# mitiko/weath3rb0i

Hardware: AMD Instinct MI355X
Metric: encode MiB/s, 64 KiB blocks, bit-exact vs CPU ref (higher is better)
Workload: dtype u32

## Files before the change

### weath3rb0i_amd/csrc/w3_predict.h

```cpp
#pragma once
#include "w3_device.h"
#include "../../include/w3hip.h"

namespace w3 {

#define W3_PF 8

#define W3_HALF_CU_LDS 81920u
template <int NW, size_t USED> struct HalfCuPad { static constexpr size_t words = (NW > 1 && USED < W3_HALF_CU_LDS) ? (W3_HALF_CU_LDS - USED + 3u) / 4u : (NW > 1 ? 0u : 1u); };
template <size_t WORDS> struct HalfCuPadDecl {
    static __device__ __forceinline__ void keep(uint64_t n) {
        __shared__ uint32_t pad_[WORDS];
        if (n == ~0ull) pad_[threadIdx.x % WORDS] = 1u;
    }
};
template <> struct HalfCuPadDecl<0> { static __device__ __forceinline__ void keep(uint64_t) {} };
#define W3_HALF_CU_PAD(NW, USED) HalfCuPadDecl<((NW) > 1 ? HalfCuPad<NW, (USED)>::words : 0u)>::keep(a.n);

struct PredictArgs {
    const uint8_t *in;
    uint64_t n;
    uint32_t block_size, nblocks;
    uint4 *P;
    const uint2 *keys;
// ... 29 lines not shown
}

template <int H>
__device__ __forceinline__ void match_windows(uint32_t w16, uint64_t M[8]) {
    uint64_t X[16];
#pragma unroll
    for (int b = 1; b < 16; b++) {
        if (b >= 1 && b <= 7 + H) {
            const bool mybit = (w16 >> b) & 1u;
            const uint64_t B = __ballot(mybit);
            X[b] = mybit ? B : ~B;
        }
    }
    if constexpr (H == 8) {
        uint64_t A2[15], A4[13];
#pragma unroll
        for (int b = 1; b <= 14; b++) A2[b] = X[b] & X[b + 1];
#pragma unroll
        for (int b = 1; b <= 12; b++) A4[b] = A2[b] & A2[b + 2];
#pragma unroll
        for (int j = 0; j < 8; j++) M[j] = A4[8 - j] & A4[12 - j];
    } else {
#pragma unroll
        for (int j = 0; j < 8; j++) {
            uint64_t m = ~0ull;
#pragma unroll
            for (int k = 0; k < H; k++) m &= X[8 - j + k];
            M[j] = m;
        }
    }
}

template <int H>
__device__ __forceinline__ void match_keys(uint2 k8, uint64_t M[8]) {
#pragma unroll
    for (int j = 0; j < 8; j++) {
        const uint32_t key = ((j < 4 ? k8.x : k8.y) >> (8 * (j & 3))) & 0xFFu;
        uint32_t mlo = 0xFFFFFFFFu, mhi = 0xFFFFFFFFu;
#pragma unroll
        for (int k = 0; k < H; k++) {
            const uint32_t sm = (uint32_t)__builtin_amdgcn_sbfe((int)key, k, 1);
            const uint64_t B = __ballot(sm != 0u);
            mlo &= ~((uint32_t)B ^ sm);
            mhi &= ~((uint32_t)(B >> 32) ^ sm);
        }
        M[j] = ((uint64_t)mhi << 32) | mlo;
    }
}

__device__ __forceinline__ uint32_t mbcnt64(uint64_t m) {
    return __builtin_amdgcn_mbcnt_hi((uint32_t)(m >> 32), __builtin_amdgcn_mbcnt_lo((uint32_t)m, 0u));
}

template <bool GROUPED>
__device__ __forceinline__ void rank_round(uint32_t c0, const uint32_t key[8], const uint64_t M[8], uint64_t seg, bool valid, bool rd,
                                           uint32_t *tbl, uint32_t p[8], uint32_t fin[8], uint32_t &wmask) {
    __asm__ volatile("" ::: "memory");
    const uint64_t gt = lane_gt_mask();
    const int lane = threadIdx.x & 63;
    wmask = 0u;
    uint32_t basev[8];
#pragma unroll
    for (int j = 0; j < 8; j++) basev[j] = tbl[j * 256 + key[j]];
#pragma unroll
    for (int j = 0; j < 8; j++) {
        const uint64_t Mj = M[j] & seg;
        const uint32_t bit = (c0 >> (7 - j)) & 1u;
        const uint64_t ones = __ballot(bit) & Mj;
        uint32_t base = basev[j];
        if constexpr (GROUPED) base = rd ? base : 0u;
        const uint32_t b0 = base & 0xFFFFu, b1 = base >> 16;
        const uint32_t n1l = mbcnt64(ones), n0l = mbcnt64(Mj) - n1l;
        uint32_t s0 = b0 + n0l, s1 = b1 + n1l;
        const bool last = valid && (Mj & gt) == 0ull;
        uint32_t f0 = s0 + (bit ^ 1u), f1 = s1 + bit;
        uint64_t satm = __ballot(last && (f0 >= 65535u || f1 >= 65535u));
        uint32_t f = f0 | (f1 << 16);
        while (satm) {
            const int k = __ffsll((long long)satm) - 1;
            const uint64_t Mc = readlane_u64(Mj, k);
            const uint64_t Oc = readlane_u64(ones, k);
            uint32_t st = readlane_u32(base, k);
            uint64_t it = Mc;
            while (it) {
                const int m = __ffsll((long long)it) - 1;
                it &= it - 1;
                if (lane == m) { s0 = st & 0xFFFFu; s1 = st >> 16; }
                st = counter_update_packed(st, (uint32_t)(Oc >> m) & 1u);
            }
            if (lane == k) f = st;
            satm &= satm - 1;
        }
        p[j] = counter_p(s0, s1);
        fin[j] = f;
        wmask |= last ? (1u << j) : 0u;
    }
    if constexpr (!GROUPED) {
#pragma unroll
        for (int j = 0; j < 8; j++)
            if ((wmask >> j) & 1u) tbl[j * 256 + key[j]] = fin[j];
        __asm__ volatile("" ::: "memory");
    }
}

#define W3_ATOMIC_LIM 65400u
#ifndef W3_ATOMIC_MAXSEG
#define W3_ATOMIC_MAXSEG 4u
#endif
typedef uint16_t w3_u16x2 __attribute__((ext_vector_type(2)));

__device__ __forceinline__ void atomic_round(uint32_t *tbl, uint32_t c0, const uint32_t key[8], bool on, uint32_t v[8]) {
#pragma unroll
    for (int j = 0; j < 8; j++) {
        const uint32_t inc = on ? (((c0 >> (7 - j)) & 1u) ? 0x10000u : 1u) : 0u;
        v[j] = __hip_atomic_fetch_add(&tbl[j * 256 + key[j]], inc, __ATOMIC_RELAXED, __HIP_MEMORY_SCOPE_WORKGROUP);
    }
}
__device__ __forceinline__ bool atomic_round_hot(const uint32_t v[8]) {
    w3_u16x2 m = __builtin_bit_cast(w3_u16x2, v[0]);
#pragma unroll
    for (int j = 1; j < 8; j++) m = __builtin_elementwise_max(m, __builtin_bit_cast(w3_u16x2, v[j]));
    return __ballot(max((uint32_t)m.x, (uint32_t)m.y) >= W3_ATOMIC_LIM) != 0ull;
}

__host__ __device__ __forceinline__ uint32_t lds_order_hash(uint32_t wave, uint32_t round, uint32_t lane) {
    uint32_t x = (wave * 64u + round) * 64u + lane + 0x9E3779B9u;
    x ^= x >> 16; x *= 0x7FEB352Du; x ^= x >> 15; x *= 0x846CA68Bu; x ^= x >> 16;
    return x;
}
__host__ __device__ __forceinline__ uint32_t lds_order_key(uint32_t wave, uint32_t h) {
    const uint32_t kind = wave & 3u;
    return kind == 0 ? 77u : kind == 1 ? (h & 7u) * 32u + 1u : kind == 2 ? (h & 255u) : (h & 2047u);
}
__global__ void __launch_bounds__(64) k_lds_order_selftest(uint32_t *old) {
    __shared__ uint32_t tbl[2048];
    const uint32_t lane = threadIdx.x;
    for (uint32_t i = lane; i < 2048u; i += 64u) tbl[i] = 0u;
    __builtin_amdgcn_wave_barrier();
    for (uint32_t r = 0; r < 32u; r++) {
        const uint32_t h = lds_order_hash(blockIdx.x, r, lane);
        old[(blockIdx.x * 32u + r) * 64u + lane] =
            __hip_atomic_fetch_add(&tbl[lds_order_key(blockIdx.x, h)], (h >> 20) & 1u ? 0x10000u : 1u, __ATOMIC_RELAXED, __HIP_MEMORY_SCOPE_WORKGROUP);
    }
}

__device__ __forceinline__ uint4 pack_p(const uint32_t p[8]) {
    return make_uint4(p[0] | (p[1] << 16), p[2] | (p[3] << 16), p[4] | (p[5] << 16), p[6] | (p[7] << 16));
}

__device__ __forceinline__ uint32_t mix_pair(uint32_t cur, uint32_t nw) {
    const uint32_t c_lo = cur & 0xFFFFu, c_hi = cur >> 16, n_lo = nw & 0xFFFFu, n_hi = nw >> 16;
    const uint32_t lo = opinion_dist(n_lo) > opinion_dist(c_lo) ? n_lo : c_lo;
    const uint32_t hi = opinion_dist(n_hi) > opinion_dist(c_hi) ? n_hi : c_hi;
    return lo | (hi << 16);
// ... 56 lines not shown
            uint2 k8 = make_uint2(0, 0);
            if constexpr (KEYS) k8 = st_k[rr * 64u + lane];
            uint32_t c0 = 0, key[8], p[8];
            if constexpr (KEYS) {
                c0 = valid ? w : 0u;
#pragma unroll
                for (int j = 0; j < 8; j++) key[j] = ((j < 4 ? k8.x : k8.y) >> (8 * (j & 3))) & KM;
            } else {
                const uint32_t wv = valid ? w : 0u;
                c0 = wv & 0xFFu;
#pragma unroll
                for (int j = 0; j < 8; j++) key[j] = ((wv & 0xFFFFu) >> (8 - j)) & KM;
            }
            if (!exact) {
                uint32_t v[8];
                __asm__ volatile("" ::: "memory");
                atomic_round(tbl, c0, key, valid, v);
                __asm__ volatile("" ::: "memory");
                if ((a.dbg_flags & 8u) && base == 64u && (a.fault_block == 0xFFFFFFFFu || a.fault_block == b)) v[0] = (uint32_t)__shfl_xor((int)v[0], 1, 64);
#pragma unroll
                for (int j = 0; j < 8; j++) p[j] = counter_p_packed(v[j]);
                exact = atomic_round_hot(v);
            } else {
                uint64_t M[8];
                if constexpr (KEYS) match_keys<H>(valid ? k8 : make_uint2(0, 0), M);
                else match_windows<H>((valid ? w : 0u) & 0xFFFFu, M);
                const uint64_t seg = __ballot(valid);
                uint32_t fin[8], wm;
                rank_round<false>(c0, key, M, seg, valid, true, tbl, p, fin, wm);
            }
            {
                uint4 *dst = valid ? a.P + (off + i) : a.sink + lane;
                *dst = pack_p(p);
            }
          }
        }
    }
}

__device__ __forceinline__ uint32_t wave_excl_scan_u32(uint32_t v, uint32_t *total) {
    const int lane = threadIdx.x & 63;
    uint32_t inc = v;
#pragma unroll
    for (int d = 1; d < 64; d <<= 1) {
        uint32_t o = __shfl_up(inc, d, 64);
        if (lane >= d) inc += o;
    }
    *total = __shfl(inc, 63, 64);
    return inc - v;
}


template <int NPASS, bool C2ONLY = false>
__device__ __forceinline__ void partition_hist(const uint8_t *blk, uint32_t len, uint32_t first, uint32_t *hist) {
    const int lane = threadIdx.x & 63;
    const uint64_t gt = lane_gt_mask();
    if (lane < 16 * NPASS) hist[lane] = 0u;
    __builtin_amdgcn_wave_barrier();
    uint32_t wn[W3_PF];
    const uint32_t last = len - 1u;
#pragma unroll
    for (int r = 0; r < W3_PF; r++) wn[r] = load_window(blk, min(r * 64u + lane, last), first);
    for (uint32_t base = 0; base < len; base += 64u * W3_PF) {
        uint32_t wc[W3_PF];
#pragma unroll
        for (int r = 0; r < W3_PF; r++) wc[r] = wn[r];
// ... 724 lines not shown
```

### weath3rb0i_amd/csrc/w3_twophase.h

```cpp
#pragma once
#include <hip/hip_runtime.h>

#include <algorithm>
#include <cstdlib>
#include <string>
#include <type_traits>
#include <vector>

#include "w3_apm.h"
#include "w3_coder.h"
#include "w3_coder4.h"
#include "w3_coder5.h"
#include "w3_predict.h"
#include "w3_predict_wave.h"
#include "w3_slot.h"
#include "w3_slot2.h"
#include "w3_spec.h"
#include "w3_tables_plan.h"

static inline const char *w3_tune_env(const char *name) {
#ifdef W3_TUNING
    return getenv(name);
#else
    (void)name;
    return nullptr;
#endif
}

enum { W3_VAR_NO_LDS_ATOMICS = 1, W3_VAR_PARTITION4 = 2, W3_VAR_NO_CHAINED_PARTITION = 4, W3_VAR_CM_UNSTAGED = 8, W3_VAR_NO_SIDE_STREAM = 16,
       W3_VAR_INJECT_LDS_FAULT = 32 ,
       W3_VAR_HALF_CU = 64    ,
       W3_VAR_FULL_CU = 128   ,
       W3_VAR_SLOT_TABLE = 256  ,
       W3_VAR_SLOT_SORTED = 512 ,
       W3_VAR_DECODE_LANE = 1024 ,
       W3_VAR_AOH_DECODE_SPEC = 2048  };

#define W3_SLOT_SORTED_MAX_BLOCKS 7000u

enum { W3_EV_PREDICT = 0, W3_EV_CODER = 1, W3_EV_PACK = 2, W3_EV_TOTAL = 3, W3_EV_APM = 4, W3_EV_SLOT = 5, W3_EV_ACHASH = 6,
       W3_EV_PART0 = 7 , W3_EV_RANK0 = 11 , W3_EV_SMALL = 15,
       W3_EV_SLOTS = 16 };
#define W3_NEV (2 * W3_EV_SLOTS)

struct TwoPhaseOptions {
    int coder_mode = 0;
    uint32_t acc_limit = 46;
    uint32_t variant = 0;
    uint32_t slot_budget_mb = 0;
    int verify = 1;
    uint32_t tune = 0;
    uint32_t fault_block = 0xFFFFFFFFu;
    uint32_t fault_kernels = 1u;
    int debug_stamps = 0;
};

struct TwoPhaseWs {
    void *P = nullptr, *keys = nullptr, *perm = nullptr, *redo = nullptr, *streams = nullptr, *rec = nullptr, *splits = nullptr;
    size_t P_cap = 0, keys_cap = 0, perm_cap = 0, redo_cap = 0, streams_cap = 0, rec_cap = 0, splits_cap = 0;
    w3::MixArgs mix{};
    bool P_valid = false;
    void *dbg = nullptr;
    bool achash_timed = false;
    hipEvent_t ev_pred_done = nullptr;
    int lds_order = -1;
    const int16_t *stretch = nullptr;
    const uint16_t *squash = nullptr;
    const uint2 *st = nullptr;
    const w3_huff_table *huff = nullptr;
    uint32_t *out_bits = nullptr;
    void *rec_w[4] = {nullptr, nullptr, nullptr, nullptr}, *perm_w[4] = {nullptr, nullptr, nullptr, nullptr}, *splits_w[4] = {nullptr, nullptr, nullptr, nullptr};
    size_t rec_w_cap[4] = {0, 0, 0, 0}, perm_w_cap[4] = {0, 0, 0, 0}, splits_w_cap[4] = {0, 0, 0, 0};
    int wide1_slot = -1;
    hipStream_t side = nullptr;
    struct PredictState {
        bool forked = false, lds_atomics = false;
        int n_def = 0, n_small_def = 0, n_live = 0;
        struct Deferred { w3::PredictArgs pa; int cls; uint32_t grid_rank; } deferred[4];
        uint64_t bytes = 0, slot_stride = 0;
        w3::SlotArgs sa;
    } pst;
    uint32_t *order_fault = nullptr;
    uint32_t *apm_oob = nullptr;
    bool half_cu = false;
    int n_wide = 0; bool small_timed = false;
    hipEvent_t ev_fork = nullptr, ev_join[4] = {nullptr, nullptr, nullptr, nullptr}, ev_small = nullptr;
    void *achash_lut = nullptr;
    size_t achash_lut_cap = 0;
    void *dummy = nullptr;
    size_t dummy_cap = 0;
    void *slot_tables = nullptr;
    size_t slot_tables_cap = 0;
    void *keys32 = nullptr; size_t keys32_cap = 0;
    void *slot_keys = nullptr; size_t slot_keys_cap = 0;
    bool slot_sorted = false;
    void *wave_tables = nullptr; size_t wave_tables_cap = 0;
    void *huff_redo = nullptr;
    size_t huff_redo_cap = 0;
    TwoPhaseOptions opt;
    uint64_t verify_calls = 0;
    TwoPhaseWs *vws = nullptr;
    void *vin = nullptr; size_t vin_cap = 0;
    bool used_lds_atomics = false;
    hipStream_t vstream = nullptr; hipEvent_t ev_v0 = nullptr, ev_v1 = nullptr;
    bool ext_streams = false;
    void release() {
        if (vws) { vws->release(); delete vws; vws = nullptr; }
        if (vin) (void)hipFree(vin);
        vin = nullptr; vin_cap = 0;
        if (vstream && !ext_streams) (void)hipStreamDestroy(vstream);
        if (ev_v0) (void)hipEventDestroy(ev_v0);
        if (ev_v1) (void)hipEventDestroy(ev_v1);
        vstream = nullptr; ev_v0 = ev_v1 = nullptr;
        if (P) (void)hipFree(P);
        if (keys) (void)hipFree(keys);
        if (perm) (void)hipFree(perm);
        if (redo) (void)hipFree(redo);
        for (int w = 0; w < 4; w++) {
            if (rec_w[w]) (void)hipFree(rec_w[w]);
            if (perm_w[w]) (void)hipFree(perm_w[w]);
            if (splits_w[w]) (void)hipFree(splits_w[w]);
            rec_w[w] = perm_w[w] = splits_w[w] = nullptr; rec_w_cap[w] = perm_w_cap[w] = splits_w_cap[w] = 0;
        }
        if (side && !ext_streams) (void)hipStreamDestroy(side);
        if (ev_fork) (void)hipEventDestroy(ev_fork);
        for (int w = 0; w < 4; w++) { if (ev_join[w]) (void)hipEventDestroy(ev_join[w]); ev_join[w] = nullptr; }
        if (ev_small) (void)hipEventDestroy(ev_small);
        ev_small = nullptr;
        side = nullptr; ev_fork = nullptr;
        if (ev_pred_done) (void)hipEventDestroy(ev_pred_done);
        ev_pred_done = nullptr;
        if (achash_lut) (void)hipFree(achash_lut);
// ... 47 lines not shown
}

static inline bool twophase_supported(const ParsedSpec &ps, size_t block_size, size_t n) {
    if (block_size > (1u << 24) || n < 8) return false;
    int n_slot = 0;
    for (int l = 0; l < ps.n_leaves; l++) n_slot += ps.leaf[l].kind == W3_NODE_SLOT_STATE;
    if (n_slot > W3_MAX_SLOT_LEAVES) return false;
    for (int l = 0; l < ps.n_leaves; l++)
        if (leaf_class(ps.leaf[l]) == LEAF_NONE) return false;
    return true;
}

#define W3_NW_SMALL 8
#define W3_NW_PART 4
#define W3_NW_RANK 6
#define W3_NW_RANK8 8
#define W3_HALF_CU_GRID 256u

template <bool KEYS, int NW = 1>
static inline void launch_small(int H, dim3 grid, hipStream_t s, const w3::PredictArgs &pa) {
    const dim3 blk(64 * NW);
    switch (H) {
    case 0: hipLaunchKernelGGL((w3::k_predict_small<0, KEYS, NW>), grid, blk, 0, s, pa); break;
    case 1: hipLaunchKernelGGL((w3::k_predict_small<1, KEYS, NW>), grid, blk, 0, s, pa); break;
    case 2: hipLaunchKernelGGL((w3::k_predict_small<2, KEYS, NW>), grid, blk, 0, s, pa); break;
    case 3: hipLaunchKernelGGL((w3::k_predict_small<3, KEYS, NW>), grid, blk, 0, s, pa); break;
    case 4: hipLaunchKernelGGL((w3::k_predict_small<4, KEYS, NW>), grid, blk, 0, s, pa); break;
    case 5: hipLaunchKernelGGL((w3::k_predict_small<5, KEYS, NW>), grid, blk, 0, s, pa); break;
    case 6: hipLaunchKernelGGL((w3::k_predict_small<6, KEYS, NW>), grid, blk, 0, s, pa); break;
    case 7: hipLaunchKernelGGL((w3::k_predict_small<7, KEYS, NW>), grid, blk, 0, s, pa); break;
    default: hipLaunchKernelGGL((w3::k_predict_small<8, KEYS, NW>), grid, blk, 0, s, pa); break;
    }
}
static inline void launch_small_shaped(const TwoPhaseWs &ws, int H, uint32_t nb, hipStream_t s, const w3::PredictArgs &pa) {
    if (ws.half_cu && (ws.opt.tune & 32u)) launch_small<false, W3_NW_SMALL>(H, dim3(std::min<uint32_t>((nb + W3_NW_SMALL - 1) / W3_NW_SMALL, 2 * W3_HALF_CU_GRID)), s, pa);
    else launch_small<false>(H, dim3(std::min<uint32_t>(nb, 256 * 20)), s, pa);
}

static inline int twophase_mix(TwoPhaseWs &ws, hipStream_t s, size_t n, std::string &err) {
    if (ws.P_valid) return W3_OK;
    int rc = tp_ensure(ws.P, ws.P_cap, n * 16, err);
    if (rc) return rc;
    ws.mix.P = (uint4 *)ws.P; ws.mix.n = n;
    hipLaunchKernelGGL(w3::k_mix, dim3(256 * 8), dim3(256), 0, s, ws.mix);
    hipError_t e = hipGetLastError();
    if (e != hipSuccess) { err = std::string("mix launch: ") + hipGetErrorString(e); return W3_E_HIP; }
    ws.P_valid = true;
    return W3_OK;
}

static inline bool twophase_lds_order_ok(TwoPhaseWs &ws, hipStream_t s) {
    if (ws.lds_order >= 0) return ws.lds_order == 1;
    ws.lds_order = 0;
    if (ws.opt.variant & W3_VAR_NO_LDS_ATOMICS) return false;
    const uint32_t waves = 64, rounds = 32, n = waves * rounds * 64;
    uint32_t *d_old = nullptr;
    if (hipMalloc(&d_old, (size_t)n * 4) != hipSuccess) { (void)hipGetLastError(); return false; }
    std::vector<uint32_t> old(n), t(2048);
    hipLaunchKernelGGL(w3::k_lds_order_selftest, dim3(waves), dim3(64), 0, s, d_old);
    bool ok = hipGetLastError() == hipSuccess && hipMemcpyAsync(old.data(), d_old, (size_t)n * 4, hipMemcpyDeviceToHost, s) == hipSuccess &&
              hipStreamSynchronize(s) == hipSuccess;
    (void)hipFree(d_old);
    if (!ok) { (void)hipGetLastError(); return false; }
    for (uint32_t w = 0; w < waves && ok; w++) {
        std::fill(t.begin(), t.end(), 0u);
        for (uint32_t r = 0; r < rounds && ok; r++)
            for (uint32_t l = 0; l < 64; l++) {
                const uint32_t h = w3::lds_order_hash(w, r, l), k = w3::lds_order_key(w, h);
                if (old[(w * rounds + r) * 64 + l] != t[k]) { ok = false; break; }
                t[k] += (h >> 20) & 1u ? 0x10000u : 1u;
            }
    }
    ws.lds_order = ok ? 1 : 0;
    return ok;
}

template <int MODE, int NW>
static inline void launch_partition8(bool fault, dim3 grid, hipStream_t s, const w3::PredictArgs &pa) {
    if (fault) hipLaunchKernelGGL((w3::k_partition8<MODE, NW, true>), grid, dim3(64 * NW), 0, s, pa);
    else hipLaunchKernelGGL((w3::k_partition8<MODE, NW>), grid, dim3(64 * NW), 0, s, pa);
}
template <int NBYTES, int NW, int PF>
static inline void launch_rank(bool fault, dim3 grid, hipStream_t s, const w3::PredictArgs &pa) {
    if (fault) hipLaunchKernelGGL((w3::k_rank_sorted<NBYTES, NW, PF, true>), grid, dim3(64 * NW), 0, s, pa);
    else hipLaunchKernelGGL((w3::k_rank_sorted<NBYTES, NW, PF>), grid, dim3(64 * NW), 0, s, pa);
}

static inline int twophase_predict_a(TwoPhaseWs &ws, hipStream_t s, const ParsedSpec &ps, const uint8_t *d_in, size_t n, size_t block_size,
                                     uint32_t nb, hipEvent_t *ev, std::string &err, bool join_all = false) {
    int rc = W3_OK;
    ws.P_valid = false;
    ws.achash_timed = false;
    const bool lds_atomics = twophase_lds_order_ok(ws, s);
    ws.used_lds_atomics = false;
    const uint32_t grid_small = std::min<uint32_t>(nb, 256 * 20);
    const uint32_t grid_wide = std::min<uint32_t>(nb, 256 * 16);
    ws.n_wide = 0; ws.small_timed = false;
    bool need_keys = false, need_perm = false;
    for (int l = 0; l < ps.n_leaves; l++) {
        int c = leaf_class(ps.leaf[l]);
        need_keys |= c == LEAF_SMALL_AC || c == LEAF_SMALL_HUFF;
        need_perm |= c == LEAF_WIDE1 || c == LEAF_WIDE2;
    }
    if (need_keys && (rc = tp_ensure(ws.keys, ws.keys_cap, n * 8, err))) return rc;
    if (need_perm) {
        int nw = 0;
        for (int l = 0; l < ps.n_leaves; l++) { const int c = leaf_class(ps.leaf[l]); nw += c == LEAF_WIDE1 || c == LEAF_WIDE2; }
        if (nw > 4) { err = "more than 4 wide Counter leaves"; return W3_E_UNSUPPORTED; }
        for (int w = 0; w < nw; w++) {
            if ((rc = tp_ensure(ws.perm_w[w], ws.perm_w_cap[w], (size_t)grid_wide * 2 * block_size * 8, err))) return rc;
            if ((rc = tp_ensure(ws.rec_w[w], ws.rec_w_cap[w], n * 8, err))) return rc;
            if ((rc = tp_ensure(ws.splits_w[w], ws.splits_w_cap[w], (size_t)nb * (W3_SLICES + 1) * 4 + 64, err))) return rc;
        }
        if (!ws.side || !ws.ev_fork) {
            bool ok = (ws.side || hipStreamCreateWithFlags(&ws.side, hipStreamNonBlocking) == hipSuccess) && hipEventCreateWithFlags(&ws.ev_fork, hipEventDisableTiming) == hipSuccess;
            for (int w = 0; w < 4 && ok; w++) ok = hipEventCreateWithFlags(&ws.ev_join[w], hipEventDisableTiming) == hipSuccess;
            ok = ok && hipEventCreateWithFlags(&ws.ev_small, hipEventDisableTiming) == hipSuccess;
            if (!ok) { (void)hipGetLastError(); err = "side stream creation failed"; return W3_E_HIP; }
        }
    }

    int live[W3_MAX_LEAVES], n_live = 0;
    for (int l = 0; l < ps.n_leaves; l++)
        if (leaf_class(ps.leaf[l]) != LEAF_FROZEN) live[n_live++] = l;
    if (n_live > 1 && (rc = tp_ensure(ws.streams, ws.streams_cap, (size_t)n_live * n * 16, err))) return rc;
    if (n_live <= 1 && (rc = tp_ensure(ws.P, ws.P_cap, n * 16, err))) return rc;

    if ((rc = tp_ensure(ws.dummy, ws.dummy_cap, 2048, err))) return rc;
// ... 85 lines not shown
                }
                hipLaunchKernelGGL(w3::k_predict_wave<true>, dim3((unsigned)waves), dim3(64), 0, s, wa);
                bytes += n * (1 + 32 + 32);
            } else {
                hipLaunchKernelGGL(w3::k_predict_wave<false>, dim3((unsigned)waves), dim3(64), 0, s, wa);
            }
            bytes += n * (8 + 16 + 8 * 16);
            hipError_t e = hipGetLastError();
            if (e != hipSuccess) { err = std::string("wave predict launch: ") + hipGetErrorString(e); return W3_E_HIP; }
            continue;
        }
        pa.hbits = nd.bits - 3;
        pa.sink = (uint4 *)ws.dummy;
        pa.maxseg = W3_ATOMIC_MAXSEG;
        if (const char *ev_ = w3_tune_env("W3_ATOMIC_MAXSEG")) pa.maxseg = (uint32_t)std::max(0, atoi(ev_));
        if (!lds_atomics) pa.dbg_flags |= 2u;
        if (ws.opt.variant & W3_VAR_INJECT_LDS_FAULT) pa.dbg_flags |= (ws.opt.fault_kernels & 7u) << 3;
        pa.fault_block = ws.opt.fault_block;
        bytes += n * 17;
        if (c == LEAF_SMALL_AC) {
            w3::HashArgs ha;
            memset(&ha, 0, sizeof ha);
            ha.in = d_in; ha.n = n; ha.block_size = (uint32_t)block_size; ha.max_bits = nd.max_bits;
            ha.hmask = (1u << (nd.bits - 3)) - 1u; ha.keys = (uint2 *)ws.keys;
            memcpy(ha.table, nd.table, sizeof ha.table);
            if ((rc = tp_ensure(ws.achash_lut, ws.achash_lut_cap, (size_t)(8u << W3_ACHASH_LUT_BITS) * 18, err))) return rc;
            ha.lut = (uint4 *)ws.achash_lut;
            ha.lut_key = (uint16_t *)((uint8_t *)ws.achash_lut + (size_t)(8u << W3_ACHASH_LUT_BITS) * 16);
            if (ev && !achash_timed) (void)hipEventRecord(ev[2 * W3_EV_ACHASH], s);
            hipLaunchKernelGGL(w3::k_achash_lut, dim3((8u << W3_ACHASH_LUT_BITS) / 256), dim3(256), 0, s, ha);
            hipLaunchKernelGGL(w3::k_achash, dim3((unsigned)((n + 255) / 256)), dim3(256), 0, s, ha);
            if (ev && !achash_timed) { (void)hipEventRecord(ev[2 * W3_EV_ACHASH + 1], s); achash_timed = true; ws.achash_timed = true; }
            pa.keys = (const uint2 *)ws.keys;
            launch_small<true>(nd.bits - 3, dim3(grid_small), s, pa);
            bytes += n * 17;
        } else if (c == LEAF_SMALL_HUFF) {
            if (!ws.huff) { err = "HuffHistory tables not staged"; return W3_E_HIP; }
            w3::HuffKeyArgs hk;
            memset(&hk, 0, sizeof hk);
            hk.in = d_in; hk.n = n; hk.block_size = (uint32_t)block_size; hk.hmask = (1u << (nd.bits - 3)) - 1u;
            hk.tb = ws.huff + nd.reserved; hk.keys = (uint2 *)ws.keys;
            if ((rc = tp_ensure(ws.huff_redo, ws.huff_redo_cap, (size_t)nb * 4, err))) return rc;
            hk.redo = (uint32_t *)ws.huff_redo; hk.nblocks = nb;
            (void)hipMemsetAsync(ws.huff_redo, 0, (size_t)nb * 4, s);
            hipLaunchKernelGGL(w3::k_huffkeys<false>, dim3((unsigned)((n + 255) / 256)), dim3(256), 0, s, hk);
            hipLaunchKernelGGL(w3::k_huffkeys_fix<false>, dim3((nb + 63u) / 64u), dim3(64), 0, s, hk);
            pa.keys = (const uint2 *)ws.keys;
            launch_small<true>(nd.bits - 3, dim3(grid_small), s, pa);
            bytes += n * 17;
        } else if (c == LEAF_SMALL) {
            if (n_small_def < 8 && (!join_all || (ws.opt.tune & 2048u))) small_def[n_small_def++] = pa;
            else {
                const bool timed = ev && !ws.small_timed;
                if (timed) { (void)hipEventRecord(ev[2 * W3_EV_SMALL], s); ws.small_timed = true; }
                launch_small_shaped(ws, nd.bits - 3, nb, s, pa);
                if (timed) (void)hipEventRecord(ev[2 * W3_EV_SMALL + 1], s);
            }
        } else {
            const int w = n_def;
            pa.perm = (uint32_t *)ws.perm_w[w];
            if (ws.opt.debug_stamps) {
                if (!ws.dbg && hipMalloc(&ws.dbg, 64) != hipSuccess) ws.dbg = nullptr;
                if (ws.dbg) { (void)hipMemsetAsync(ws.dbg, 0, 64, s); pa.dbg = (unsigned long long *)ws.dbg; }
            }
            pa.rec = (uint2 *)ws.rec_w[w]; pa.splits = (uint32_t *)ws.splits_w[w];
            pa.job_counter = (uint32_t *)ws.splits_w[w] + (size_t)nb * (W3_SLICES + 1);
            (void)hipMemsetAsync(pa.job_counter, 0, 4, sp);
            if (const char *ev_ = w3_tune_env("W3_DEBUG_NOSTORE")) pa.dbg_flags = (uint32_t)atoi(ev_) & 5u;
            if (!lds_atomics) pa.dbg_flags |= 2u;
            uint32_t rank_waves = 2048u;
            if (const char *ev_ = w3_tune_env("W3_RANK_GRID")) rank_waves = (uint32_t)std::max(64, atoi(ev_));
            const uint32_t nw_rank = (ws.opt.tune & 32768u) ? W3_NW_RANK8 : W3_NW_RANK;
            const uint32_t grid_rank = (ws.half_cu && (w == 0 || (ws.opt.tune & (32u | 64u))) && !(ws.opt.tune & 8u)) ? std::min<uint32_t>((nb * W3_SLICES + nw_rank - 1) / nw_rank, W3_HALF_CU_GRID)
                                                              : std::min<uint32_t>(nb * W3_SLICES, rank_waves);
            const bool chained = c == LEAF_WIDE2 && ws.wide1_slot >= 0 && !(ws.opt.variant & W3_VAR_NO_CHAINED_PARTITION);
            if (chained) pa.rec_src = (const uint2 *)ws.rec_w[ws.wide1_slot];
            const bool p8 = lds_atomics && !(ws.opt.variant & W3_VAR_PARTITION4);
            const uint32_t grid_p8h = std::min<uint32_t>((nb + W3_NW_PART - 1) / W3_NW_PART, 2 * W3_HALF_CU_GRID);
            const bool p8h = p8 && ws.half_cu && (ws.opt.tune & 32u);
            if (ev && w < 4) (void)hipEventRecord(ev[2 * (W3_EV_PART0 + w)], sp);
            const bool f8 = (pa.dbg_flags & 32u) != 0u;
// ... 165 lines not shown
    if (tm) tm->predict_bytes = bytes;
    if (d_P) *d_P = (const uint16_t *)ws.P;
    return W3_OK;
}

static inline int twophase_predict(TwoPhaseWs &ws, hipStream_t s, const ParsedSpec &ps, const uint8_t *d_in, size_t n, size_t block_size,
                                   uint32_t nb, bool need_P, const uint16_t **d_P, hipEvent_t *ev, w3_timing *tm, std::string &err) {
    int rc = twophase_predict_a(ws, s, ps, d_in, n, block_size, nb, ev, err, false);
    if (rc) return rc;
    return twophase_predict_b(ws, s, ps, d_in, n, block_size, nb, need_P, d_P, ev, tm, err);
}

static inline int twophase_verify(TwoPhaseWs &ws, hipStream_t s, const ParsedSpec &ps, const uint8_t *d_in, size_t n, size_t block_size,
                                  uint32_t nb, uint32_t *d_mismatch, std::string &err) {
    if (!ws.opt.verify || !ws.used_lds_atomics || nb == 0) return W3_OK;
    const uint32_t S = w3::verify_sample_size(nb, block_size, (uint32_t)std::max(1, ws.opt.verify));
    const uint32_t rot = w3::verify_rotation(ws.verify_calls, nb, S);
    const uint64_t last_off = (uint64_t)w3::verify_block(rot, S - 1u, nb, S) * block_size;
    const size_t vn = (size_t)(S - 1u) * block_size + (size_t)std::min<uint64_t>(block_size, n - last_off);
    const uint8_t *vsrc = nullptr;
    int rc;
    if (nb == 1) vsrc = d_in;
    else {
        if ((rc = tp_ensure(ws.vin, ws.vin_cap, vn, err))) return rc;
        hipLaunchKernelGGL(w3::k_gather_blocks, dim3(std::min<uint32_t>((uint32_t)((block_size + 255) / 256), 64u), S), dim3(256), 0, s,
                           d_in, (uint64_t)n, (uint32_t)block_size, nb, S, rot, (uint8_t *)ws.vin);
        vsrc = (const uint8_t *)ws.vin;
    }
    if (!ws.vws) ws.vws = new TwoPhaseWs();
    TwoPhaseWs &v = *ws.vws;
    v.opt = TwoPhaseOptions();
    v.opt.variant = (ws.opt.variant | W3_VAR_NO_LDS_ATOMICS | W3_VAR_PARTITION4 | W3_VAR_NO_SIDE_STREAM) & ~(uint32_t)W3_VAR_INJECT_LDS_FAULT;
    v.opt.verify = 0; v.opt.slot_budget_mb = ws.opt.slot_budget_mb;
    v.lds_order = 0;
    v.stretch = ws.stretch; v.squash = ws.squash; v.st = ws.st; v.huff = ws.huff;
    ParsedSpec vps;
    int map[W3_MAX_LEAVES], nmap = 0;
    int live_idx = 0;
    for (int l = 0; l < ps.n_leaves; l++) {
        const int c = leaf_class(ps.leaf[l]);
        if (c == LEAF_FROZEN) continue;
        if (c != LEAF_SLOT && c != LEAF_WAVE) { vps.leaf[vps.n_leaves++] = ps.leaf[l]; map[nmap++] = live_idx; }
        live_idx++;
    }
    vps.n_huff = ps.n_huff; vps.huff = ps.huff;
    if (vps.n_leaves == 0) return W3_OK;
    if ((rc = twophase_predict(v, s, vps, vsrc, vn, block_size, (uint32_t)((vn + block_size - 1) / block_size), false, nullptr, nullptr, nullptr, err))) return rc;
    for (int k = 0; k < nmap; k++)
        hipLaunchKernelGGL(w3::k_compare_blocks, dim3(std::min<uint32_t>((uint32_t)((block_size + 255) / 256), 64u), S), dim3(256), 0, s,
                           ws.mix.src[map[k]], v.mix.src[k], (uint64_t)n, (uint32_t)block_size, nb, S, rot, d_mismatch);
    hipError_t e = hipGetLastError();
    if (e != hipSuccess) { err = std::string("verify launch: ") + hipGetErrorString(e); return W3_E_HIP; }
    return W3_OK;
}

static inline int twophase_apm(TwoPhaseWs &ws, hipStream_t s, const ParsedSpec &ps, const uint8_t *d_in, size_t n, size_t block_size,
                               uint32_t nb, hipEvent_t *ev, w3_timing *tm, std::string &err) {
    if (ps.n_apm == 0) return W3_OK;
    if (!ws.stretch || !ws.squash) { err = "APM LUTs not staged"; return W3_E_HIP; }
    int rc = tp_ensure(ws.P, ws.P_cap, n * 16, err);
    if (rc) return rc;
    if ((rc = tp_ensure(ws.dummy, ws.dummy_cap, 2048, err))) return rc;
    if (ev) (void)hipEventRecord(ev[2 * W3_EV_APM], s);
    uint64_t bytes = 0;
    bool partitioned = false;
    for (int k = 0; k < ps.n_apm; k++) {
        w3::ApmArgs aa;
// ... 198 lines not shown
```

### weath3rb0i_amd/csrc/w3hip.hip

```cpp
#include "../../include/w3hip.h"

#include <hip/hip_runtime.h>

#include <algorithm>
#include <cstddef>
#include <cstdio>
#include <cstring>
#include <mutex>
#include <string>
#include <thread>
#include <vector>

#include "w3_spec.h"
#include "w3_huff.h"
#include "w3_generic.h"
#include "w3_cm.h"
#include "w3_decode_spec.h"
#include "w3_pack.h"
#include "w3_tables_plan.h"
#include "w3_jobs.h"
#include "w3_twophase.h"
#include "w3_selftest.h"
#include "w3_sweep.h"
#include "w3_aoh.h"
// ... 52 lines not shown
    int state = 0;
    int djob = -1, rc = W3_OK;
    uint64_t seq = 0, total = 0;
    DevBuf d_in, d_out, d_lens, d_total;
    hipEvent_t ev_d2h = nullptr;
    KeptCall call;
    size_t nb = 0, dcap = 0;
    uint8_t *out = nullptr; size_t out_cap = 0; uint32_t *block_lens = nullptr;
    w3_timing tm{};
};

struct w3_ctx {
    int device = 0;
    hipStream_t stream = nullptr;
    std::string err;
    int opt_path = W3_PATH_AUTO;
    int opt_timing = 0;
    w3_timing timing{};
    DevBuf tables, lens, total, io_in, io_out, coffs, misc, cm_luts, achash_luts, sweep;
    DevBuf aoh;
    DevBuf rg_stage, rg_meta;
    void *h_rg = nullptr; size_t h_rg_cap = 0;
    DevBuf crc_ws, crc_tab;
    DevBuf prep_ws;
    DevBuf exp_d, exp_s, exp_list, exp_stats;
    size_t exp_d_zero = 0;
    uint32_t export_epoch = 0;
    w3_export_entropy_profile exp_prof{};
    DevBuf exp_k, exp_hs;
    uint64_t crc_res[2] = {~0ull, 0};
    TwoPhaseOptions opt;
    const int16_t *stretch = nullptr; const uint16_t *squash = nullptr; const uint2 *st = nullptr;
    int lds_order = -1;
    Job jobs[W3_MAX_JOBS];
    w3_ctx() { for (int j = 0; j < W3_MAX_JOBS; j++) jobs[j].index = j; }
    hipStream_t s_pred = nullptr, s_code[W3_MAX_JOBS] = {};
    int next_job = 0, last_job = -1;
    bool pooled_streams = false;
    hipStream_t s_side = nullptr, s_verify[W3_MAX_JOBS] = {};
    struct ShardSlot { int state = 0, djob = -1; DevBuf out, lens, total; size_t nb = 0, cap = 0; KeptCall call; } ss[W3_MAX_JOBS];
    HostJob hj[W3_MAX_HOST_JOBS];
    hipStream_t s_h2d = nullptr, s_d2h = nullptr;
    hipStream_t s_h2d_own = nullptr, s_d2h_own = nullptr;
    uint64_t hseq = 0;
    uint32_t host_chunk_blocks = 0;
    uint32_t aoh_batch_blocks = 0;
    w3::VerifyCalls vcalls;
    int64_t vcall_pin = -1;
};

static uint64_t verify_call(w3_ctx *ctx, size_t n, size_t block_size) {
    return ctx->vcall_pin >= 0 ? (uint64_t)ctx->vcall_pin : ctx->vcalls.next(n, block_size);
}
struct VcallPin {
    w3_ctx *c; int64_t saved;
    VcallPin(w3_ctx *c_, uint64_t v) : c(c_), saved(c_->vcall_pin) { c->vcall_pin = (int64_t)v; }
    ~VcallPin() { c->vcall_pin = saved; }
};

#define HIPCHK(ctx, expr)                                                                       \
    do {                                                                                        \
        hipError_t e_ = (expr);                                                                 \
        if (e_ != hipSuccess) {                                                                 \
            (ctx)->err = std::string(#expr) + ": " + hipGetErrorString(e_);                     \
            return W3_E_HIP;                                                                    \
        }                                                                                       \
// ... 120 lines not shown
    if (!ctx) return W3_E_INVALID;
    if (opt != W3_OPT_TIMING && opt != W3_OPT_TUNE) { const int rc_ = jobs_idle(ctx); if (rc_) return rc_; }
    switch (opt) {
    case W3_OPT_PATH:
        if (value < W3_PATH_AUTO || value > W3_PATH_TWOPHASE) return W3_E_INVALID;
        ctx->opt_path = (int)value;
        return W3_OK;
    case W3_OPT_TIMING: ctx->opt_timing = value ? 1 : 0; return W3_OK;
    case W3_OPT_CODER:
        if (value < 0 || value > 5) return W3_E_INVALID;
        ctx->opt.coder_mode = (int)value;
        return W3_OK;
    case W3_OPT_DEBUG_STAMPS: ctx->opt.debug_stamps = value ? 1 : 0; return W3_OK;
    case W3_OPT_ACC_LIMIT:
        if (value < 19 || value > 46) return W3_E_INVALID;
        ctx->opt.acc_limit = (uint32_t)value;
        return W3_OK;
    case W3_OPT_VARIANT:
        if (value < 0 || value > 4095) return W3_E_INVALID;
        if ((value & W3_VAR_INJECT_LDS_FAULT) && !ctx->opt.verify) { ctx->err = "W3_OPT_VARIANT bit 32 (fault injection) needs W3_OPT_VERIFY on"; return W3_E_INVALID; }
        ctx->opt.variant = (uint32_t)value;
        ctx->lds_order = -1;
        return W3_OK;
    case W3_OPT_VERIFY:
        if (!value && (ctx->opt.variant & W3_VAR_INJECT_LDS_FAULT)) { ctx->err = "W3_OPT_VERIFY cannot be switched off while the fault-injection variant is set"; return W3_E_INVALID; }
        if (value < 0 || value > 256) return W3_E_INVALID;
        ctx->opt.verify = (int)value;
        return W3_OK;
    case W3_OPT_SLOT_BUDGET_MB:
        if (value < 0 || value > (1 << 20)) return W3_E_INVALID;
        ctx->opt.slot_budget_mb = (uint32_t)value;
        return W3_OK;
    case W3_OPT_TUNE:
        if (value < 0 || value > 0xFFFFF) return W3_E_INVALID;
        ctx->opt.tune = (uint32_t)value;
        return W3_OK;
    case W3_OPT_FAULT_BLOCK:
        if (value < -1 || value > 0x7FFFFFFF) return W3_E_INVALID;
        ctx->opt.fault_block = value < 0 ? 0xFFFFFFFFu : (uint32_t)value;
        return W3_OK;
    case W3_OPT_FAULT_KERNELS:
        if (value < 1 || value > 7) return W3_E_INVALID;
        ctx->opt.fault_kernels = (uint32_t)value;
        return W3_OK;
    case W3_OPT_HOST_CHUNK_BLOCKS:
        if (value < 0 || value > 0x7FFFFFFF) return W3_E_INVALID;
        ctx->host_chunk_blocks = (uint32_t)value;
        return W3_OK;
    case W3_OPT_AOH_BATCH_BLOCKS:
        if (value < 0 || value > 0x7FFFFFFF) return W3_E_INVALID;
        ctx->aoh_batch_blocks = (uint32_t)value;
        return W3_OK;
    case W3_OPT_EXPORT_EPOCH:
        if (value < 0 || value > (int64_t)W3_EXP_EPOCH_MAX || value % 1024) { ctx->err = "an export epoch is a multiple of 1 KiB, at most 2^28 bytes"; return W3_E_INVALID; }
        ctx->export_epoch = (uint32_t)value;
        return W3_OK;
    default: return W3_E_INVALID;
    }
}

extern "C" int w3_get_timing(const w3_ctx *ctx, w3_timing *out) {
    if (!ctx || !out) return W3_E_INVALID;
    *out = ctx->timing;
    return W3_OK;
}

extern "C" size_t w3_max_compressed_size(size_t n, size_t block_size) {
// ... 280 lines not shown
    float ms = 0.f;
    if (hipEventElapsedTime(&ms, ev[2 * slot], ev[2 * slot + 1]) != hipSuccess) { (void)hipGetLastError(); return 0.f; }
    return ms;
}

static void collect_timing(hipEvent_t *ev, const TwoPhaseWs &ws, bool has_apm, bool has_slot, bool packed, w3_timing &t) {
    t.predict_ms = elapsed_ev(ev, W3_EV_PREDICT); t.coder_ms = elapsed_ev(ev, W3_EV_CODER);
    if (has_apm) t.apm_ms = elapsed_ev(ev, W3_EV_APM);
    if (has_slot) t.slot_ms = elapsed_ev(ev, W3_EV_SLOT);
    if (ws.achash_timed) t.achash_ms = elapsed_ev(ev, W3_EV_ACHASH);
    t.n_wide = (uint32_t)std::min(ws.n_wide, 4);
    for (int w = 0; w < ws.n_wide && w < 4; w++) { t.part_ms[w] = elapsed_ev(ev, W3_EV_PART0 + w); t.rank_ms[w] = elapsed_ev(ev, W3_EV_RANK0 + w); }
    if (ws.small_timed) t.small_ms = elapsed_ev(ev, W3_EV_SMALL);
    t.pack_ms = packed ? elapsed_ev(ev, W3_EV_PACK) : 0.f;
    t.total_ms = elapsed_ev(ev, W3_EV_TOTAL);
}

static int stage_huff_job(w3_ctx *ctx, Job &J, hipStream_t s, const ParsedSpec &ps) {
    J.tp.huff = nullptr;
    if (!ps.n_huff) return W3_OK;
    ENSURE(ctx, J.huff, sizeof(w3_huff_table) * W3_MAX_HUFF);
    HIPCHK(ctx, hipMemcpyAsync(J.huff.p, ps.huff, sizeof(w3_huff_table) * ps.n_huff, hipMemcpyHostToDevice, s));
    HIPCHK(ctx, hipStreamSynchronize(s));
    J.tp.huff = (const w3_huff_table *)J.huff.p;
    return W3_OK;
}

static int stage_huff(w3_ctx *ctx, hipStream_t s, const ParsedSpec &ps) { return stage_huff_job(ctx, ctx->jobs[0], s, ps); }

static void hand_options(w3_ctx *ctx, Job &J, bool two) {
    J.tp.opt = ctx->opt;
    if (J.index) J.tp.opt.debug_stamps = 0;
    J.tp.stretch = ctx->stretch; J.tp.squash = ctx->squash; J.tp.st = ctx->st;
    J.tp.lds_order = ctx->lds_order;
    if (two && ctx->lds_order < 0) { (void)twophase_lds_order_ok(J.tp, ctx->stream); ctx->lds_order = J.tp.lds_order; }
}

static void use_ballot_rounds(w3_ctx *ctx) {
    ctx->opt.variant |= W3_VAR_NO_LDS_ATOMICS; ctx->lds_order = 0;
    for (auto &J : ctx->jobs) { J.tp.opt.variant |= W3_VAR_NO_LDS_ATOMICS; J.tp.lds_order = 0; }
}

static int attach_aux_streams(w3_ctx *ctx, Job &J) {
    if (!ctx->s_side) {
        ctx->s_side = stream_pool().take(ctx->device * 8L + 2);
        if (!ctx->s_side) HIPCHK(ctx, hipStreamCreateWithFlags(&ctx->s_side, hipStreamNonBlocking));
    }
    hipStream_t &sv = ctx->s_verify[J.index];
    if (!sv) {
        sv = stream_pool().take(ctx->device * 8L + 3);
        if (!sv) {
            int lo_p = 0, hi_p = 0;
            HIPCHK(ctx, hipDeviceGetStreamPriorityRange(&lo_p, &hi_p));
            HIPCHK(ctx, hipStreamCreateWithPriority(&sv, hipStreamNonBlocking, lo_p));
        }
    }
    J.tp.side = ctx->s_side; J.tp.vstream = sv; J.tp.ext_streams = true;
    return W3_OK;
}

static int stage_cm_luts(w3_ctx *ctx, hipStream_t s) {
    CmArgs lut;
    const int rc = cm_luts(ctx, s, lut);
    if (!rc) { ctx->stretch = lut.stretch; ctx->squash = lut.squash; ctx->st = lut.st; }
    return rc;
}

// ... 2650 lines not shown
```

Before: 14270.

## Size small predict grids to resident occupancy; add opt-in split-table kernel

Small-leaf predict launches now get a grid sized from the occupancy API times the CU count, cached per kernel form and H, instead of a fixed 256*20 blocks. That applies to both the default one-wave kernel and the keyed kernels. A new two-wave kernel, which splits the 8 counter tables between waves (4 each), is added behind a new tune bit and is not on by default. The grid sizing is meant to avoid oversubscribing or undersubscribing the persistent block loops, at the cost of one occupancy query per configuration.

```diff
diff --git a/weath3rb0i_amd/csrc/w3_predict.h b/weath3rb0i_amd/csrc/w3_predict.h
--- a/weath3rb0i_amd/csrc/w3_predict.h
+++ b/weath3rb0i_amd/csrc/w3_predict.h
@@ -85,6 +85,19 @@
 }
 
 template <int H>
+__device__ __forceinline__ uint64_t match_window1(uint32_t wj) {
+    uint32_t mlo = 0xFFFFFFFFu, mhi = 0xFFFFFFFFu;
+#pragma unroll
+    for (int k = 0; k < H; k++) {
+        const uint32_t sm = (uint32_t)__builtin_amdgcn_sbfe((int)wj, k, 1);
+        const uint64_t B = __ballot(sm != 0u);
+        mlo &= ~((uint32_t)B ^ sm);
+        mhi &= ~((uint32_t)(B >> 32) ^ sm);
+    }
+    return ((uint64_t)mhi << 32) | mlo;
+}
+
+template <int H>
 __device__ __forceinline__ void match_keys(uint2 k8, uint64_t M[8]) {
 #pragma unroll
     for (int j = 0; j < 8; j++) {
@@ -105,20 +118,20 @@
     return __builtin_amdgcn_mbcnt_hi((uint32_t)(m >> 32), __builtin_amdgcn_mbcnt_lo((uint32_t)m, 0u));
 }
 
-template <bool GROUPED>
-__device__ __forceinline__ void rank_round(uint32_t c0, const uint32_t key[8], const uint64_t M[8], uint64_t seg, bool valid, bool rd,
-                                           uint32_t *tbl, uint32_t p[8], uint32_t fin[8], uint32_t &wmask) {
+template <bool GROUPED, int NJ = 8>
+__device__ __forceinline__ void rank_round(uint32_t c0, const uint32_t key[NJ], const uint64_t M[NJ], uint64_t seg, bool valid, bool rd,
+                                           uint32_t *tbl, uint32_t p[NJ], uint32_t fin[NJ], uint32_t &wmask) {
     __asm__ volatile("" ::: "memory");
     const uint64_t gt = lane_gt_mask();
     const int lane = threadIdx.x & 63;
     wmask = 0u;
-    uint32_t basev[8];
-#pragma unroll
-    for (int j = 0; j < 8; j++) basev[j] = tbl[j * 256 + key[j]];
-#pragma unroll
-    for (int j = 0; j < 8; j++) {
+    uint32_t basev[NJ];
+#pragma unroll
+    for (int j = 0; j < NJ; j++) basev[j] = tbl[j * 256 + key[j]];
+#pragma unroll
+    for (int j = 0; j < NJ; j++) {
         const uint64_t Mj = M[j] & seg;
-        const uint32_t bit = (c0 >> (7 - j)) & 1u;
+        const uint32_t bit = (c0 >> (NJ - 1 - j)) & 1u;
         const uint64_t ones = __ballot(bit) & Mj;
         uint32_t base = basev[j];
         if constexpr (GROUPED) base = rd ? base : 0u;
@@ -150,7 +163,7 @@
     }
     if constexpr (!GROUPED) {
 #pragma unroll
-        for (int j = 0; j < 8; j++)
+        for (int j = 0; j < NJ; j++)
             if ((wmask >> j) & 1u) tbl[j * 256 + key[j]] = fin[j];
         __asm__ volatile("" ::: "memory");
     }
@@ -162,17 +175,19 @@
 #endif
 typedef uint16_t w3_u16x2 __attribute__((ext_vector_type(2)));
 
-__device__ __forceinline__ void atomic_round(uint32_t *tbl, uint32_t c0, const uint32_t key[8], bool on, uint32_t v[8]) {
-#pragma unroll
-    for (int j = 0; j < 8; j++) {
-        const uint32_t inc = on ? (((c0 >> (7 - j)) & 1u) ? 0x10000u : 1u) : 0u;
+template <int NJ = 8>
+__device__ __forceinline__ void atomic_round(uint32_t *tbl, uint32_t c0, const uint32_t key[NJ], bool on, uint32_t v[NJ]) {
+#pragma unroll
+    for (int j = 0; j < NJ; j++) {
+        const uint32_t inc = on ? (((c0 >> (NJ - 1 - j)) & 1u) ? 0x10000u : 1u) : 0u;
         v[j] = __hip_atomic_fetch_add(&tbl[j * 256 + key[j]], inc, __ATOMIC_RELAXED, __HIP_MEMORY_SCOPE_WORKGROUP);
     }
 }
-__device__ __forceinline__ bool atomic_round_hot(const uint32_t v[8]) {
+template <int NJ = 8>
+__device__ __forceinline__ bool atomic_round_hot(const uint32_t v[NJ]) {
     w3_u16x2 m = __builtin_bit_cast(w3_u16x2, v[0]);
 #pragma unroll
-    for (int j = 1; j < 8; j++) m = __builtin_elementwise_max(m, __builtin_bit_cast(w3_u16x2, v[j]));
+    for (int j = 1; j < NJ; j++) m = __builtin_elementwise_max(m, __builtin_bit_cast(w3_u16x2, v[j]));
     return __ballot(max((uint32_t)m.x, (uint32_t)m.y) >= W3_ATOMIC_LIM) != 0ull;
 }
 
@@ -295,6 +310,84 @@
             {
                 uint4 *dst = valid ? a.P + (off + i) : a.sink + lane;
                 *dst = pack_p(p);
+            }
+          }
+        }
+    }
+}
+
+template <int H>
+__global__ void __launch_bounds__(128) __attribute__((amdgpu_waves_per_eu(8, 8))) k_predict_small_split(PredictArgs a) {
+    __shared__ uint32_t tbl_[2][4 * 256];
+    __shared__ uint16_t st_w_[2][W3_PF * 64];
+    static_assert(sizeof(tbl_) + sizeof(st_w_) <= 10240, "16 blocks per CU");
+    const int lane = threadIdx.x & 63;
+    const uint32_t wv = (uint32_t)__builtin_amdgcn_readfirstlane((int)(threadIdx.x >> 6));
+    uint32_t *tbl = tbl_[wv];
+    uint16_t *st_w = st_w_[wv];
+    const uint32_t wsh = 4u - 4u * wv;
+    constexpr uint32_t KM = (1u << H) - 1u;
+    uint8_t *Pw = reinterpret_cast<uint8_t *>(a.P) + 8u * wv;
+    uint2 *sink = reinterpret_cast<uint2 *>(a.sink) + threadIdx.x;
+    for (uint32_t b = blockIdx.x; b < a.nblocks; b += gridDim.x) {
+        const uint64_t off = (uint64_t)b * a.block_size;
+        const uint32_t len = (uint32_t)((a.n - off) < a.block_size ? (a.n - off) : a.block_size);
+        const uint8_t *blk = a.in + off;
+#pragma unroll
+        for (int k = 0; k < 16; k++) tbl[k * 64 + lane] = 0u;
+        __builtin_amdgcn_wave_barrier();
+        bool exact = (a.dbg_flags & 2u) != 0u;
+        const uint32_t first = window_head(off, 3u);
+        const uint32_t last = len - 1u;
+        uint32_t nw[W3_PF];
+#pragma unroll
+        for (int r = 0; r < W3_PF; r++) nw[r] = load_window(blk, min((uint32_t)(r * 64 + lane), last), first);
+        for (uint32_t bbase = 0; bbase < len; bbase += 64u * W3_PF) {
+            __asm__ volatile("" ::: "memory");
+            __builtin_amdgcn_wave_barrier();
+#pragma unroll
+            for (int r = 0; r < W3_PF; r++) st_w[r * 64 + lane] = (uint16_t)(((nw[r] & 0xFFFFu) >> wsh) & 0xFFFu);
+            __asm__ volatile("" ::: "memory");
+            __builtin_amdgcn_wave_barrier();
+#pragma unroll
+            for (int r = 0; r < W3_PF; r++) nw[r] = load_window(blk, min(bbase + (uint32_t)((W3_PF + r) * 64 + lane), last), first);
+#pragma unroll 1
+          for (uint32_t rr = 0; rr < W3_PF; rr++) {
+            const uint32_t base = bbase + rr * 64u;
+            if (base >= len) break;
+            const uint32_t i = base + lane;
+            const bool valid = i < len;
+            const uint32_t w = valid ? (uint32_t)st_w[rr * 64u + lane] : 0u;
+            const uint32_t c0 = w & 0xFu;
+            uint2 pp = make_uint2(0u, 0u);
+            if (!exact) {
+                uint32_t key[4], p[4], v[4];
+#pragma unroll
+                for (int j = 0; j < 4; j++) key[j] = (w >> (4 - j)) & KM;
+                __asm__ volatile("" ::: "memory");
+                atomic_round<4>(tbl, c0, key, valid, v);
+                __asm__ volatile("" ::: "memory");
+                if ((a.dbg_flags & 8u) && wv == 0u && base == 64u && (a.fault_block == 0xFFFFFFFFu || a.fault_block == b)) v[0] = (uint32_t)__shfl_xor((int)v[0], 1, 64);
+#pragma unroll
+                for (int j = 0; j < 4; j++) p[j] = counter_p_packed(v[j]);
+                exact = atomic_round_hot<4>(v);
+                pp = make_uint2(p[0] | (p[1] << 16), p[2] | (p[3] << 16));
+            } else {
+                const uint64_t seg = __ballot(valid);
+#pragma unroll 1
+                for (uint32_t j = 0; j < 4u; j++) {
+                    const uint32_t wj = w >> (4u - j);
+                    const uint32_t key1 = wj & KM, bit1 = (w >> (3u - j)) & 1u;
+                    const uint64_t M1 = match_window1<H>(wj);
+                    uint32_t p1, fin1, wm;
+                    rank_round<false, 1>(bit1, &key1, &M1, seg, valid, true, tbl + j * 256u, &p1, &fin1, wm);
+                    const uint32_t ph = p1 << (16u * (j & 1u));
+                    if (j < 2u) pp.x |= ph; else pp.y |= ph;
+                }
+            }
+            {
+                uint2 *dst = valid ? reinterpret_cast<uint2 *>(Pw + 16u * (off + i)) : sink;
+                *dst = pp;
             }
           }
         }
diff --git a/weath3rb0i_amd/csrc/w3_twophase.h b/weath3rb0i_amd/csrc/w3_twophase.h
--- a/weath3rb0i_amd/csrc/w3_twophase.h
+++ b/weath3rb0i_amd/csrc/w3_twophase.h
@@ -54,6 +54,8 @@
     uint32_t fault_kernels = 1u;
     int debug_stamps = 0;
 };
+
+struct ResidentGrids { uint32_t wg[3][9] = {}; };
 
 struct TwoPhaseWs {
     void *P = nullptr, *keys = nullptr, *perm = nullptr, *redo = nullptr, *streams = nullptr, *rec = nullptr, *splits = nullptr;
@@ -98,6 +100,7 @@
     void *huff_redo = nullptr;
     size_t huff_redo_cap = 0;
     TwoPhaseOptions opt;
+    ResidentGrids *grids = nullptr;
     uint64_t verify_calls = 0;
     TwoPhaseWs *vws = nullptr;
     void *vin = nullptr; size_t vin_cap = 0;
@@ -211,9 +214,43 @@
     default: hipLaunchKernelGGL((w3::k_predict_small<8, KEYS, NW>), grid, blk, 0, s, pa); break;
     }
 }
+enum { W3_SMALL_ONE_WAVE = 0, W3_SMALL_KEYED = 1, W3_SMALL_SPLIT = 2 };
+#define W3_TUNE_SMALL_SPLIT 1048576u
+template <int FORM, int H>
+static inline auto small_kernel() -> void (*)(w3::PredictArgs) {
+    if constexpr (FORM == W3_SMALL_SPLIT) return w3::k_predict_small_split<H>;
+    else if constexpr (FORM == W3_SMALL_KEYED) return w3::k_predict_small<H, true, 1>;
+    else return w3::k_predict_small<H, false, 1>;
+}
+template <int FORM>
+static inline void launch_small_resident(const TwoPhaseWs &ws, int H, uint32_t nb, hipStream_t s, const w3::PredictArgs &pa) {
+    void (*k)(w3::PredictArgs) = nullptr;
+    switch (H) {
+    case 0: k = small_kernel<FORM, 0>(); break;
+    case 1: k = small_kernel<FORM, 1>(); break;
+    case 2: k = small_kernel<FORM, 2>(); break;
+    case 3: k = small_kernel<FORM, 3>(); break;
+    case 4: k = small_kernel<FORM, 4>(); break;
+    case 5: k = small_kernel<FORM, 5>(); break;
+    case 6: k = small_kernel<FORM, 6>(); break;
+    case 7: k = small_kernel<FORM, 7>(); break;
+    default: k = small_kernel<FORM, 8>(); H = 8; break;
+    }
+    const int threads = FORM == W3_SMALL_SPLIT ? 128 : 64;
+    uint32_t own = 0u, &resident = ws.grids ? ws.grids->wg[FORM][H] : own;
+    if (!resident) {
+        int per_cu = 0, dev = 0, cus = 0;
+        if (hipOccupancyMaxActiveBlocksPerMultiprocessor(&per_cu, k, threads, 0) == hipSuccess && hipGetDevice(&dev) == hipSuccess &&
+            hipDeviceGetAttribute(&cus, hipDeviceAttributeMultiprocessorCount, dev) == hipSuccess && per_cu > 0 && cus > 0)
+            resident = (uint32_t)per_cu * (uint32_t)cus;
+        else { (void)hipGetLastError(); resident = 256u * 20u; }
+    }
+    hipLaunchKernelGGL(k, dim3(std::min<uint32_t>(nb, resident)), dim3(threads), 0, s, pa);
+}
 static inline void launch_small_shaped(const TwoPhaseWs &ws, int H, uint32_t nb, hipStream_t s, const w3::PredictArgs &pa) {
     if (ws.half_cu && (ws.opt.tune & 32u)) launch_small<false, W3_NW_SMALL>(H, dim3(std::min<uint32_t>((nb + W3_NW_SMALL - 1) / W3_NW_SMALL, 2 * W3_HALF_CU_GRID)), s, pa);
-    else launch_small<false>(H, dim3(std::min<uint32_t>(nb, 256 * 20)), s, pa);
+    else if (ws.opt.tune & W3_TUNE_SMALL_SPLIT) launch_small_resident<W3_SMALL_SPLIT>(ws, H, nb, s, pa);
+    else launch_small_resident<W3_SMALL_ONE_WAVE>(ws, H, nb, s, pa);
 }
 
 static inline int twophase_mix(TwoPhaseWs &ws, hipStream_t s, size_t n, std::string &err) {
@@ -272,7 +309,6 @@
     ws.achash_timed = false;
     const bool lds_atomics = twophase_lds_order_ok(ws, s);
     ws.used_lds_atomics = false;
-    const uint32_t grid_small = std::min<uint32_t>(nb, 256 * 20);
     const uint32_t grid_wide = std::min<uint32_t>(nb, 256 * 16);
     ws.n_wide = 0; ws.small_timed = false;
     bool need_keys = false, need_perm = false;
@@ -424,7 +460,7 @@
             hipLaunchKernelGGL(w3::k_achash, dim3((unsigned)((n + 255) / 256)), dim3(256), 0, s, ha);
             if (ev && !achash_timed) { (void)hipEventRecord(ev[2 * W3_EV_ACHASH + 1], s); achash_timed = true; ws.achash_timed = true; }
             pa.keys = (const uint2 *)ws.keys;
-            launch_small<true>(nd.bits - 3, dim3(grid_small), s, pa);
+            launch_small_resident<W3_SMALL_KEYED>(ws, nd.bits - 3, nb, s, pa);
             bytes += n * 17;
         } else if (c == LEAF_SMALL_HUFF) {
             if (!ws.huff) { err = "HuffHistory tables not staged"; return W3_E_HIP; }
@@ -438,7 +474,7 @@
             hipLaunchKernelGGL(w3::k_huffkeys<false>, dim3((unsigned)((n + 255) / 256)), dim3(256), 0, s, hk);
             hipLaunchKernelGGL(w3::k_huffkeys_fix<false>, dim3((nb + 63u) / 64u), dim3(64), 0, s, hk);
             pa.keys = (const uint2 *)ws.keys;
-            launch_small<true>(nd.bits - 3, dim3(grid_small), s, pa);
+            launch_small_resident<W3_SMALL_KEYED>(ws, nd.bits - 3, nb, s, pa);
             bytes += n * 17;
         } else if (c == LEAF_SMALL) {
             if (n_small_def < 8 && (!join_all || (ws.opt.tune & 2048u))) small_def[n_small_def++] = pa;
@@ -670,7 +706,7 @@
     v.opt = TwoPhaseOptions();
     v.opt.variant = (ws.opt.variant | W3_VAR_NO_LDS_ATOMICS | W3_VAR_PARTITION4 | W3_VAR_NO_SIDE_STREAM) & ~(uint32_t)W3_VAR_INJECT_LDS_FAULT;
     v.opt.verify = 0; v.opt.slot_budget_mb = ws.opt.slot_budget_mb;
-    v.lds_order = 0;
+    v.lds_order = 0; v.grids = ws.grids;
     v.stretch = ws.stretch; v.squash = ws.squash; v.st = ws.st; v.huff = ws.huff;
     ParsedSpec vps;
     int map[W3_MAX_LEAVES], nmap = 0;
diff --git a/weath3rb0i_amd/csrc/w3hip.hip b/weath3rb0i_amd/csrc/w3hip.hip
--- a/weath3rb0i_amd/csrc/w3hip.hip
+++ b/weath3rb0i_amd/csrc/w3hip.hip
@@ -108,6 +108,7 @@
     TwoPhaseOptions opt;
     const int16_t *stretch = nullptr; const uint16_t *squash = nullptr; const uint2 *st = nullptr;
     int lds_order = -1;
+    ResidentGrids grids;
     Job jobs[W3_MAX_JOBS];
     w3_ctx() { for (int j = 0; j < W3_MAX_JOBS; j++) jobs[j].index = j; }
     hipStream_t s_pred = nullptr, s_code[W3_MAX_JOBS] = {};
@@ -294,7 +295,7 @@
         ctx->opt.slot_budget_mb = (uint32_t)value;
         return W3_OK;
     case W3_OPT_TUNE:
-        if (value < 0 || value > 0xFFFFF) return W3_E_INVALID;
+        if (value < 0 || value > 0x1FFFFF) return W3_E_INVALID;
         ctx->opt.tune = (uint32_t)value;
         return W3_OK;
     case W3_OPT_FAULT_BLOCK:
@@ -641,7 +642,7 @@
     J.tp.opt = ctx->opt;
     if (J.index) J.tp.opt.debug_stamps = 0;
     J.tp.stretch = ctx->stretch; J.tp.squash = ctx->squash; J.tp.st = ctx->st;
-    J.tp.lds_order = ctx->lds_order;
+    J.tp.lds_order = ctx->lds_order; J.tp.grids = &ctx->grids;
     if (two && ctx->lds_order < 0) { (void)twophase_lds_order_ok(J.tp, ctx->stream); ctx->lds_order = J.tp.lds_order; }
 }
 
```

Result: no change. 14220 (-0.3%).
